# arangrhie/merfin

Measured on AMD Instinct MI355X. Metric: k-mers evaluated/sec (-hist, k=21), higher is better.
Workload: dtype u64 k-mers / u32 counts / f64 K*

## Files before the change

### merfin_amd/csrc/mfx_device.h

```cpp
#pragma once
#include "mfx_internal.h"
#include "mfx_kernels.h"

__device__ __forceinline__ uint64_t mfx_hash64(uint64_t x) {
  x ^= x >> 33; x *= 0xff51afd7ed558ccdULL;
  x ^= x >> 33; x *= 0xc4ceb9fe1a85ec53ULL;
  x ^= x >> 33;
  return x;
}

__device__ __forceinline__ uint32_t mfx_range32(uint64_t x, uint64_t n) {
  const uint32_t n32 = (uint32_t)n;
  const uint64_t t = (uint64_t)(uint32_t)(x >> 32) * n32 + (uint64_t)__umulhi((uint32_t)x, n32);
  return (uint32_t)(t >> 32);
}

__device__ __forceinline__ uint64_t mfx_field_mask(uint32_t nbits) { return nbits >= 64u ? ~0ull : (1ull << nbits) - 1ull; }
__device__ __forceinline__ uint64_t mfx_bits_at(const uint64_t *w, uint64_t bit, uint32_t nbits, uint64_t mask) {
  const uint64_t i = bit >> 6;
  const uint32_t sh = (uint32_t)bit & 63u;
  uint64_t x = w[i] >> sh;
  if (sh + nbits > 64u) x |= w[i + 1] << (64u - sh);
  return x & mask;
}
// ... 36 lines not shown

constexpr uint32_t MFX_TILE_BYTES  = MFX_TILE + 64;
constexpr uint32_t MFX_TILE_CHUNKS = MFX_TILE_BYTES / 16;
constexpr uint32_t MFX_TILE_WORDS  = MFX_TILE_BYTES / 32;

struct mfx_tile_lds {
  uint64_t codes[MFX_TILE_WORDS + 1];
  uint32_t valid[MFX_TILE_WORDS + 1];
};

__device__ __forceinline__ void mfx_pack16(uint4 v, uint32_t &codes, uint32_t &valid) {
  uint32_t w[4] = {v.x, v.y, v.z, v.w};
  codes = 0;
  valid = 0;
#pragma unroll
  for (int q = 0; q < 4; ++q) {
#pragma unroll
    for (int b = 0; b < 4; ++b) {
      uint32_t c = (w[q] >> (8 * b)) & 0xffu;
      uint32_t u = (c & 0xDFu) - 0x41u;
      uint32_t ok = (u < 32u) ? ((0x00080045u >> u) & 1u) : 0u;
      int i = q * 4 + b;
      codes |= ((c >> 1) & 3u) << (30 - 2 * i);
      valid |= ok << (15 - i);
    }
  }
}

__device__ __forceinline__ void mfx_tile_fill(mfx_tile_lds &L, const uint8_t *__restrict__ src) {
  uint32_t *c32 = reinterpret_cast<uint32_t *>(L.codes);
  uint16_t *v16 = reinterpret_cast<uint16_t *>(L.valid);
  for (uint32_t ch = threadIdx.x; ch < MFX_TILE_CHUNKS; ch += MFX_BLOCK) {
    uint4 v = *reinterpret_cast<const uint4 *>(src + 16ull * ch);
    uint32_t codes, valid;
    mfx_pack16(v, codes, valid);
    c32[ch ^ 1] = codes;
    v16[ch ^ 1] = (uint16_t)valid;
  }
}

__device__ __forceinline__ void mfx_tile_fill_packed(mfx_tile_lds &L, const uint64_t *__restrict__ codes, const uint32_t *__restrict__ valid) {
  for (uint32_t i = threadIdx.x; i < MFX_TILE_WORDS; i += MFX_BLOCK) {
    L.codes[i] = codes[i];
    L.valid[i] = valid[i];
  }
}

__device__ __forceinline__ uint64_t mfx_wave_sum(uint64_t v) {
#pragma unroll
  for (int o = 32; o > 0; o >>= 1) v += __shfl_down(v, o, 64);
  return v;
}

__device__ __forceinline__ void mfx_block_sum3(uint64_t &a, uint64_t &b, uint64_t &c, uint64_t (*scratch)[3]) {
  a = mfx_wave_sum(a); b = mfx_wave_sum(b); c = mfx_wave_sum(c);
  uint32_t wave = threadIdx.x >> 6, lane = threadIdx.x & 63;
  __syncthreads();
  if (lane == 0) { scratch[wave][0] = a; scratch[wave][1] = b; scratch[wave][2] = c; }
  __syncthreads();
  if (threadIdx.x == 0) {
    a = b = c = 0;
    for (uint32_t w = 0; w < MFX_BLOCK / 64; ++w) { a += scratch[w][0]; b += scratch[w][1]; c += scratch[w][2]; }
  }
}


#ifndef MFX_V_LDS_DIET
#define MFX_V_LDS_DIET 1
#endif
struct mfx_hist_lds {
  uint32_t hist[2 * MFX_NB_LDS];
  uint32_t rk[MFX_MAXP_LDS];
#if !MFX_V_LDS_DIET
  double   pr[MFX_MAXP_LDS];
#endif
  uint16_t bin[MFX_KLUT * MFX_KLUT];
#if !MFX_V_LDS_DIET
  double   term[MFX_KLUT * MFX_KLUT];
#endif
  uint32_t lut_ok;
  uint32_t wl_n;
  uint64_t next[2];
  uint64_t tot[2];
  uint64_t red[MFX_BLOCK / 64][3];
  double   dred[MFX_BLOCK];
};

__device__ __forceinline__ void mfx_hist_lds_init(mfx_hist_lds &H, const mfx_kstar_args &ka) {
  const uint32_t tid = threadIdx.x;
  for (uint32_t i = tid; i < 2 * MFX_NB_LDS; i += MFX_BLOCK) H.hist[i] = 0;
  if (tid == 0) H.lut_ok = 1u;
  __syncthreads();
  for (uint32_t v = tid; v < MFX_MAXP_LDS; v += MFX_BLOCK) {
    double rk, pr;
    mfx_getK_core(ka.peak, ka.n_prob, ka.probK, ka.probP, v, rk, pr);
    if (!(rk >= 0.0 && rk < 4294967296.0 && rk == (double)(uint32_t)rk)) H.lut_ok = 0u;
    H.rk[v] = (uint32_t)rk;
#if !MFX_V_LDS_DIET
    H.pr[v] = pr;
#endif
  }
  for (uint32_t i = tid; i < MFX_KLUT * MFX_KLUT; i += MFX_BLOCK) {
    uint32_t h = i / MFX_KLUT, l = i % MFX_KLUT;
    uint32_t b = (h >= 1 && l >= 1 && h >= l) ? mfx_bin_index((double)h, (double)l) : 0u;
    H.bin[i] = (uint16_t)b;
#if !MFX_V_LDS_DIET
    H.term[i] = (h >= 1 && l >= 1 && h > l) ? mfx_overcopy_term((double)l, (double)h, 1.0) : 0.0;
#endif
  }
  __syncthreads();
}

__device__ __forceinline__ void mfx_ovf_add(uint64_t *ovf, uint64_t key, uint64_t amount) {
  unsigned long long *cnt = reinterpret_cast<unsigned long long *>(ovf) + 2, *keys = cnt + MFX_OVF_SLOTS;
  uint64_t x = key * 0x9E3779B97F4A7C15ull;
  uint32_t h = (uint32_t)(x >> 40) & (MFX_OVF_SLOTS - 1u);
  for (uint32_t probe = 0; probe < MFX_OVF_PROBES; ++probe) {
    unsigned long long cur = __hip_atomic_load(&keys[h], __ATOMIC_RELAXED, __HIP_MEMORY_SCOPE_AGENT);
    if (cur == ~0ull) {
      cur = atomicCAS(&keys[h], ~0ull, (unsigned long long)key);
      if (cur == ~0ull) { atomicAdd(reinterpret_cast<unsigned long long *>(ovf), 1ull); cur = key; }
    }
    if (cur == key) { atomicAdd(&cnt[h], (unsigned long long)amount); return; }
    h = (h + 1u) & (MFX_OVF_SLOTS - 1u);
  }
  atomicAdd(reinterpret_cast<unsigned long long *>(ovf) + 1, (unsigned long long)amount);
}

__device__ __forceinline__ void mfx_ovf_record(const mfx_kstar_args &ka, bool under, uint32_t idx) {
  const uint64_t key = (under ? 0ull : (1ull << 63)) | idx;
  const uint32_t lane = threadIdx.x & 63u;
  uint64_t todo = __ballot(1);
  while (todo) {
    const int leader = __ffsll((unsigned long long)todo) - 1;
    const uint64_t lk = ((uint64_t)(uint32_t)__shfl((int)(key >> 32), leader, 64) << 32) | (uint32_t)__shfl((int)(uint32_t)key, leader, 64);
    const uint64_t same = __ballot(key == lk) & todo;
    if ((int)lane == leader) {
      const uint64_t n = (uint64_t)__popcll(same);
      mfx_ovf_add(ka.ovf, key, n);
      atomicAdd((unsigned long long *)&ka.counts[2ull * ka.nbins + 2], (unsigned long long)n);
    }
    todo &= ~same;
  }
}

template <class Counter>
__device__ __forceinline__ bool mfx_hist_eval(mfx_hist_lds &H, const mfx_kstar_args &ka, bool lut_ok, uint32_t readV,
                                              uint32_t asmV, Counter &n_over0, double &kover) {
  double readK, prob;
  uint32_t rki = 0xffffffffu;
  if (lut_ok && readV < MFX_MAXP_LDS) {
#if MFX_V_LDS_DIET
    rki = H.rk[readV]; prob = 1.0; readK = (double)rki;
#else
    rki = H.rk[readV]; prob = H.pr[readV]; readK = (double)rki;
#endif
  } else {
    mfx_getK_core(ka.peak, ka.n_prob, ka.probK, ka.probP, readV, readK, prob);
  }
  const double asmK = (double)asmV;
  if (readK == 0) return true;
  const bool under = asmK > readK;
  uint32_t idx;
  if (rki < MFX_KLUT && asmV < MFX_KLUT && asmV >= 1) {
    const uint32_t hi = under ? asmV : rki, lo = under ? rki : asmV;
    idx = H.bin[hi * MFX_KLUT + lo];
// ... 77 lines not shown
```

### merfin_amd/csrc/mfx_kernels.hip

```cpp
#include "mfx_internal.h"
#include "mfx_kernels.h"
#include "mfx_device.h"
#include "mfx_place.h"
#include "mfx_track.h"
#define MFX_REGIONS_DEVICE
#include "mfx_regions.h"
#include "mfx_spectrum.h"

#include <stdlib.h>
#include <algorithm>

__device__ __forceinline__ uint64_t mfx_revcomp(uint64_t fwd, int k) {
  uint64_t x = __brevll(fwd) >> (64 - 2 * k);
  x = ((x & 0x5555555555555555ULL) << 1) | ((x >> 1) & 0x5555555555555555ULL);
  uint64_t mask = (~0ULL) >> (64 - 2 * k);
  return (x ^ 0xAAAAAAAAAAAAAAAAULL) & mask;
}


constexpr uint32_t MFX_MZ_REGION = 4;
constexpr uint32_t MFX_MAX_LINES = 512;

struct mfx_probe {
  uint32_t lineA, lineB;
// ... 1555 lines not shown
      }
      if (have) x = make_uint2((r_rv < c.minV || r_rv > c.maxV) ? 0u : r_rv, r_av);
#pragma unroll
      for (int j = 0; j < B; ++j)
        if (sj == j) { rv[j] = x.x; av[j] = x.y; st[j] = 0xffu; }
    }
  }
  return defer;
}

template <class KmerAt, class Eval, class Push1>
__device__ __forceinline__ void mfx_lane_flush(const mfx_table_view &c, mfx_mailbox &M, uint32_t &nq, KmerAt kmer_at, Eval eval, Push1 push1, unsigned long long *dbg = nullptr) {
  const uint32_t tid = threadIdx.x, sub16 = (tid & 7u) << 4, lane = tid & 63u, wbase = tid & ~63u;
  const uint32_t n = nq;
  nq = 0u;
  if (n == 0u) return;
  mfx_wave_handoff();
  constexpr uint32_t STEPS = 4;
  auto tail_pass = [&](bool second) {
    for (uint32_t q0 = 0; q0 < n; q0 += 8u * STEPS) {
      uint4 sl[STEPS];
      uint32_t fl[STEPS];
      bool act[STEPS];
#pragma unroll
      for (uint32_t sp = 0; sp < STEPS; ++sp) {
        const uint32_t e = q0 + 8u * sp + (lane >> 3);
        sl[sp] = make_uint4(0u, 0u, 0u, 0u);
        act[sp] = false;
        fl[sp] = 0u;
        if (e < n) {
          const uint2 lw = *reinterpret_cast<const uint2 *>(reinterpret_cast<const uint32_t *>(&M.rec[wbase + e]) + 2);
          fl[sp] = lw.y;
          act[sp] = lw.x != MFX_REC_FOUND && (!second || (lw.y & 3u) == 2u);
          if (act[sp]) sl[sp] = *reinterpret_cast<const uint4 *>(reinterpret_cast<uint64_t>(c.slots) + ((uint64_t)lw.x << 7) + sub16);
        }
      }
      mfx_wave_handoff();
#pragma unroll
      for (uint32_t sp = 0; sp < STEPS; ++sp) {
        const uint32_t e = q0 + 8u * sp + (lane >> 3);
        if (act[sp]) {
          uint32_t *rec = reinterpret_cast<uint32_t *>(&M.rec[wbase + e]);
          const uint2 kk = *reinterpret_cast<const uint2 *>(rec);
          if (sl[sp].y == 0xffffffffu || sl[sp].w == 0xffffffffu) rec[3] = (fl[sp] & ~3u) | 1u;
          if (sl[sp].y == kk.y && ((sl[sp].x ^ kk.x) >> 22) == 0u) { rec[0] = sl[sp].x; rec[2] = MFX_REC_FOUND; }
          else if (sl[sp].w == kk.y && ((sl[sp].z ^ kk.x) >> 22) == 0u) { rec[0] = sl[sp].z; rec[2] = MFX_REC_FOUND; }
        }
      }
    }
    mfx_wave_handoff();
  };
  tail_pass(false);
  const bool mine = lane < n;
  uint4 r = make_uint4(0u, 0u, MFX_REC_FOUND, 0u);
  if (mine) r = M.rec[wbase + lane];
  const bool full = mine && r.z != MFX_REC_FOUND && (r.w & 3u) != 1u;
  if (__any(full)) {
    if (full) {
      uint32_t *rec = reinterpret_cast<uint32_t *>(&M.rec[wbase + lane]);
      mfx_probe pr;
      pr.lineA = pr.lineB = r.z;
      rec[2] = (uint32_t)mfx_probe_line(c, pr, 1u);
      rec[3] = (r.w & ~3u) | 2u;
      if (c.quot) rec[1] = r.y | (1u << (MFX_Q_DSHIFT + 22 - 32));
      if (dbg) atomicAdd(&dbg[1], 1ull);
    }
    mfx_wave_handoff();
    tail_pass(true);
    if (full) {
      const uint4 r2 = M.rec[wbase + lane];
      r.x = r2.x; r.w = r2.w;
      if (r2.z == MFX_REC_FOUND) r.z = MFX_REC_FOUND;
    }
  }
  bool have = r.z == MFX_REC_FOUND;
  uint32_t lo = r.x;
  uint64_t fk = (((uint64_t)r.y << 32) | r.x) >> 22;
  if (c.quot) fk &= (1ull << MFX_Q_DSHIFT) - 1ull;
  const bool scan = mine && !have && (r.w & 3u) == 2u;
  const bool satd = mine && have && (((lo >> 11) & MFX_CSAT) == MFX_CSAT || (lo & MFX_CSAT) == MFX_CSAT);
  bool listed = false;
  if (__any(scan || satd)) {
    if (dbg && (scan || satd)) atomicAdd(&dbg[scan ? 3 : 2], 1ull);
    listed = push1(scan || satd, (scan || satd) ? (c.quot ? kmer_at(r.w >> 4) : fk) : 0ull, scan ? r.z : lo, scan ? 1u : 2u) && (scan || satd);
  }
  if (mine && !listed) {
    bool beyond = false;
    if (scan) {
      if (dbg) atomicAdd(&dbg[5], 1ull);
      const uint2 fd = mfx_c_find_lean(c, fk, r.z, 2u, beyond);
      have = fd.x != 0u;
      lo = fd.y;
    }
    uint32_t r_rv = (lo >> 11) & MFX_CSAT, r_av = lo & MFX_CSAT;
    const bool sat = have && (r_rv == MFX_CSAT || r_av == MFX_CSAT);
    if (sat || beyond) {
      const uint2 sx = mfx_side_lookup_lean(c, c.quot ? kmer_at(r.w >> 4) : fk);
      if (beyond) { r_rv = sx.x; r_av = sx.y; have = true; }
      else { if (r_rv == MFX_CSAT) r_rv = sx.x; if (r_av == MFX_CSAT) r_av = sx.y; }
    }
    uint32_t o_rv = 0u, o_av = 0u;
    if (have) { o_rv = (r_rv < c.minV || r_rv > c.maxV) ? 0u : r_rv; o_av = r_av; }
    eval(o_rv, o_av);
  }
  mfx_wave_handoff();
}

template <int B>
struct mfx_key_from_array {
  const uint64_t (&key)[B];
  __device__ __forceinline__ uint64_t operator()(int sj) const {
    uint64_t k = 0;
#pragma unroll
    for (int j = 0; j < B; ++j) if (j == sj) k = key[j];
    return k;
  }
};

#ifndef MFX_V_LANEPROBE
#define MFX_V_LANEPROBE 1
#endif

template <int B>
__device__ __forceinline__ void mfx_compact_lookup(const mfx_table_view &t, mfx_mailbox &M, const uint64_t (&key)[B], const uint64_t (&krc)[B],
                                                   const bool (&ok)[B], uint32_t (&rv)[B], uint32_t (&av)[B]) {
#if MFX_V_LANEPROBE
  uint64_t fkey[B];
  uint32_t line[B], b0[B];
#pragma unroll
  for (int j = 0; j < B; ++j) {
    fkey[j] = key[j]; line[j] = 0u; b0[j] = 0u;
    if (ok[j]) { const mfx_probe pr = mfx_home(t, key[j]); fkey[j] = pr.fkey; line[j] = pr.lineA; b0[j] = pr.b0; }
  }
  (void)mfx_lane_lookup8<B>(t, M, fkey, ok, rv, av, line, b0, mfx_key_from_array<B>{key});
#else
  mfx_group_lookup8<B>(t, M, key, krc, ok, rv, av);
#endif
}
#define MFX_COMPACT_LOOKUP(t, MB, key, krc, ok, rv, av) mfx_compact_lookup<MFX_BATCH>(t, MB, key, krc, ok, rv, av)

__device__ __forceinline__ bool mfx_tile_kmer(const mfx_tile_lds &L, int k, uint32_t p, uint64_t &fwd) {
  uint32_t w = p >> 5, o = p & 31;
  uint64_t w0 = L.codes[w], w1 = L.codes[w + 1];
  uint32_t sh = 2 * o;
  uint64_t hi = (w0 << sh) | ((w1 >> 1) >> (63 - sh));
  fwd = hi >> (64 - 2 * k);
  uint64_t vv = (((uint64_t)L.valid[w] << 32) | L.valid[w + 1]) << o;
  return (vv >> (64 - k)) == ((~0ULL) >> (64 - k));
}

#ifndef MFX_V_MIN2LEVEL
#define MFX_V_MIN2LEVEL 1
#endif
typedef unsigned short mfx_us2 __attribute__((ext_vector_type(2)));
__device__ __forceinline__ uint32_t mfx_pk_min_u16(uint32_t a, uint32_t b) {
  return __builtin_bit_cast(uint32_t, __builtin_elementwise_min(__builtin_bit_cast(mfx_us2, a), __builtin_bit_cast(mfx_us2, b)));
}
__device__ __forceinline__ uint32_t mfx_mod_pack(uint32_t order, uint32_t q) { return ((order << 7) | q) | (((order << 7) | (127u - q)) << 16); }

template <int B>
__device__ __forceinline__ void mfx_wave_mod_halo(const mfx_table_view &c, const mfx_tile_lds &L, uint32_t p0, uint32_t (&halo)[2]) {
  const int t = c.mz_t;
  const uint32_t H = (uint32_t)(c.k - t), per = 64u / H;
  const uint32_t lane = threadIdx.x & 63u;
  const uint32_t jj = lane / H, ii = lane - H * jj;
#pragma unroll
  for (uint32_t ps = 0; ps < 2u; ++ps) {
    halo[ps] = 0xffffffffu;
    const uint32_t el = ps * per + jj;
    if (ps * per < (uint32_t)B && jj < per && el < (uint32_t)B) {
      const uint32_t q = p0 - lane + el * MFX_BLOCK + 64u + ii, wd = q >> 5, o = q & 31u, sh = 2u * o;
      const uint64_t w0 = L.codes[wd], w1 = L.codes[wd + 1];
      const uint32_t a = (uint32_t)(((w0 << sh) | ((w1 >> 1) >> (63u - sh))) >> (64 - 2 * t));
      const uint32_t b = (uint32_t)mfx_revcomp((uint64_t)a, t);
      halo[ps] = mfx_mod_pack(mfx_tmer_order(a < b ? a : b), 64u + ii);
    }
  }
}

__device__ __forceinline__ uint32_t mfx_wave_mod_line(const mfx_table_view &c, uint32_t *mw, const uint32_t (&halo)[2], int j, uint64_t f, uint64_t r,
                                                      uint32_t &b0, uint64_t &fkey) {
  const int k = c.k, t = c.mz_t, w = c.mz_w, m = k - w + 1, npos = k - t + 1;
  const uint32_t lane = threadIdx.x & 63u, tmask = (1u << (2 * t)) - 1u;
  const uint32_t H = (uint32_t)(k - t), per = 64u / H;
  const uint64_t mmask = (~0ULL) >> (64 - 2 * m);
  const uint32_t a = (uint32_t)(f >> (2 * (k - t))) & tmask, b = (uint32_t)r & tmask;
  const uint32_t hsrc = (uint32_t)j < per ? halo[0] : halo[1];
  const uint32_t hv = (uint32_t)__shfl((int)hsrc, (int)(H * ((uint32_t)j < per ? (uint32_t)j : (uint32_t)j - per) + lane), 64);
  mfx_wave_handoff();
  mw[lane] = mfx_mod_pack(mfx_tmer_order(a < b ? a : b), lane);
  if (lane <= H) mw[64u + lane] = lane < H ? hv : 0xffffffffu;
  mfx_wave_handoff();
  uint32_t v = 0xffffffffu;
#if MFX_V_MIN2LEVEL
  {
    const int g1 = npos >= 26 ? 6 : npos >= 10 ? 4 : npos >= 5 ? 3 : 2, g2 = (npos + g1 - 1) / g1;
    uint32_t a0 = 0xffffffffu, a1 = 0xffffffffu;
#pragma unroll
    for (int i = 0; i < 6; ++i)
      if (i < g1) { a0 = mfx_pk_min_u16(a0, mw[lane + (uint32_t)i]); a1 = mfx_pk_min_u16(a1, mw[(lane <= (uint32_t)(npos - g1) ? 64u + lane : lane) + (uint32_t)i]); }
    mfx_wave_handoff();
    mw[lane] = a0;
    if (lane <= (uint32_t)(npos - g1)) mw[64u + lane] = a1;
    mfx_wave_handoff();
#pragma unroll
    for (int j = 0; j < 7; ++j)
      if (j < g2) v = mfx_pk_min_u16(v, mw[lane + (uint32_t)(j * g1 < npos - g1 ? j * g1 : npos - g1)]);
  }
#else
#pragma unroll
  for (int i = 0; i < 28; ++i)
    if (i < npos) v = mfx_pk_min_u16(v, mw[lane + (uint32_t)i]);
#endif
  const bool fwd = f <= r;
  const uint32_t q = fwd ? (v & 127u) : 127u - ((v >> 16) & 127u);
  const uint32_t xf = q - lane, jf = xf % (uint32_t)w;
  const uint64_t ma = (f >> (2 * ((uint32_t)w - 1u - jf))) & mmask, mb = (r >> (2 * jf)) & mmask;
  const uint32_t xc = fwd ? xf : (uint32_t)(k - t) - xf;
  uint32_t line;
  fkey = fwd ? f : r;
  if (c.quot) {
    const uint32_t jc = fwd ? jf : 3u - jf;
    const uint64_t ac = fwd ? ma : mb, bc = fwd ? mb : ma;
    const uint32_t e = (uint32_t)(((fkey >> (2 * (m + 3 - (int)jc))) << (2 * (3 - (int)jc))) | (fkey & ((1ull << (2 * (3 - (int)jc))) - 1ull)));
    mfx_q_place(c, ac < bc ? ac : bc, bc < ac ? 1u : 0u, jc, e, xc, line, b0, fkey);
  } else {
    const bool lt = ma < mb, keep = lt || (fwd && ma == mb);
    mfx_mod_place(lt ? ma : mb, keep ? jf : (uint32_t)w - 1u - jf, c.nlines, line, b0, xc);
  }
  return line;
}


#ifndef MFX_V_BATCH
#define MFX_V_BATCH 4
#endif
constexpr int MFX_BATCH = MFX_V_BATCH;

#ifndef MFX_V_MINBLOCKS
#define MFX_V_MINBLOCKS 4
#endif
#ifndef MFX_V_MINBLOCKS_K21
#define MFX_V_MINBLOCKS_K21 7
#endif
#ifndef MFX_V_BATCH_K21
#define MFX_V_BATCH_K21 2
#endif
#ifndef MFX_V_MINBLOCKS_K31
#define MFX_V_MINBLOCKS_K31 6
#endif
#ifndef MFX_V_BATCH_K31
#define MFX_V_BATCH_K31 2
#endif
#ifndef MFX_V_MINBLOCKS_GEN
#define MFX_V_MINBLOCKS_GEN 4
#endif
#ifndef MFX_V_BATCH_GEN
#define MFX_V_BATCH_GEN 4
#endif
#ifndef MFX_V_DEFER_K21
#define MFX_V_DEFER_K21 0
#endif
#ifndef MFX_V_DEFER_K31
#define MFX_V_DEFER_K31 1
#endif
#ifndef MFX_V_KFXLDS_K21
#define MFX_V_KFXLDS_K21 1
#endif
constexpr uint32_t MFX_KFX_BASE = 32u;
#ifndef MFX_V_BUCKET2_K21
#define MFX_V_BUCKET2_K21 0
#endif
#ifndef MFX_V_BUCKET2_K31
#define MFX_V_BUCKET2_K31 1
#endif
template <bool CANON, bool COMPACT, int KF> struct mfx_hist_tune { static constexpr int blocks = MFX_V_MINBLOCKS, batch = MFX_V_BATCH, defer = 0, kfxlds = 0, bucket2 = 0; };
template <> struct mfx_hist_tune<true, true, 21> { static constexpr int blocks = MFX_V_MINBLOCKS_K21, batch = MFX_V_BATCH_K21, defer = MFX_V_DEFER_K21, kfxlds = MFX_V_KFXLDS_K21, bucket2 = MFX_V_BUCKET2_K21; };
#ifndef MFX_V_KFXLDS_K31
#define MFX_V_KFXLDS_K31 0
#endif
template <> struct mfx_hist_tune<true, true, 31> { static constexpr int blocks = MFX_V_MINBLOCKS_K31, batch = MFX_V_BATCH_K31, defer = MFX_V_DEFER_K31, kfxlds = MFX_V_KFXLDS_K31, bucket2 = MFX_V_BUCKET2_K31; };
template <> struct mfx_hist_tune<true, true, 0> { static constexpr int blocks = MFX_V_MINBLOCKS_GEN, batch = MFX_V_BATCH_GEN, defer = 0, kfxlds = 0, bucket2 = 0; };
template <bool CANON, bool COMPACT, int KF, int WF, int TF, bool DBG = false>
__global__ __launch_bounds__(MFX_BLOCK, (mfx_hist_tune<CANON, COMPACT, KF>::blocks)) void mfx_hist_kernel(mfx_hist_args a) {
  constexpr int BT = mfx_hist_tune<CANON, COMPACT, KF>::batch;
  __shared__ mfx_tile_lds L;
  __shared__ mfx_mailbox MB;
  __shared__ mfx_hist_lds H;

  const uint32_t tid = threadIdx.x;
  if (KF) { a.t.k = KF; a.t.mz_w = WF; a.t.mz_t = TF; a.t.quot = KF > MFX_MAX_K_DIRECT ? 1 : 0; }
  const int k = KF ? KF : a.t.k;
  const mfx_kstar_args &ka = a.ks;
  mfx_hist_lds_init(H, ka);
  const bool lut_ok = H.lut_ok != 0u;

  uint32_t n_valid = 0, n_missing = 0, n_over0 = 0;
  if (tid == 0) { H.tot[0] = H.tot[1] = 0; H.wl_n = 0u; }
  uint64_t *c_glob = ka.counts + 2ull * ka.nbins;
  uint64_t *c_kasm = c_glob + 3, *c_kmis = c_kasm + ka.ncontigs;

  const uint32_t none = 0xffffffffu;
  uint32_t c = none;
  uint64_t li = blockIdx.x;
  for (uint32_t it = 0; li < a.n_logical; ++it) {
    if (tid == 0)
      H.next[it & 1] = (uint64_t)gridDim.x + atomicAdd((unsigned long long *)a.tile_ctr, 1ull);
    const uint64_t tile = a.part_n == 1 ? a.tile_begin + li
                                         : ((((li >> a.part_shift) * a.part_n + a.part_rank) << a.part_shift) | (li & ((1ull << a.part_shift) - 1ull)));
    const uint32_t cn = a.tile_contig[tile];
    if (cn != c) {
      if (c != none) {
        uint64_t x = n_valid, y = n_missing, z = 0;
        mfx_block_sum3(x, y, z, H.red);
        if (tid == 0 && (x | y)) {
          atomicAdd((unsigned long long *)&c_kasm[c], x);
          atomicAdd((unsigned long long *)&c_kmis[c], y);
          H.tot[0] += x;
          H.tot[1] += y;
        }
        n_valid = n_missing = 0;
      }
      c = cn;
    }
    const uint64_t pos0 = (tile - a.tile_start[c]) * MFX_TILE;
    const uint64_t clen = a.contig_len[c];
    const uint32_t n = (clen - pos0 < MFX_TILE) ? (uint32_t)(clen - pos0) : MFX_TILE;
    const uint8_t *src = a.bases + a.contig_off[c] + pos0;

    if (a.codes) {
      const uint64_t w0 = (a.contig_off[c] + pos0) >> 5;
      mfx_tile_fill_packed(L, a.codes + w0, a.valid + w0);
    } else {
      mfx_tile_fill(L, src);
    }
    __syncthreads();

    uint64_t kfx = 0;
    constexpr bool kfx_lds = mfx_hist_tune<CANON, COMPACT, KF>::kfxlds != 0 && COMPACT && CANON && KF != 0 && TF != 0;
    constexpr uint32_t mb_cap = kfx_lds ? MFX_KFX_BASE : 64u;
    static_assert(!(mfx_hist_tune<CANON, COMPACT, KF>::kfxlds != 0 && mfx_hist_tune<CANON, COMPACT, KF>::defer != 0),
                  "kfxlds packs 16 terms and a count of at most 16 into one LDS word per lane: the deferred probe lets a lane evaluate more than its own 16 k-mers of a tile");
    static_assert(MFX_TILE / MFX_BLOCK <= 16, "the packed koverCpy word (56-bit sum, 8-bit count) holds 16 evaluations per lane and tile");
    unsigned long long *const kfxw = reinterpret_cast<unsigned long long *>(&MB.rec[(tid & ~63u) + MFX_KFX_BASE]) + (tid & 63u);
    if (kfx_lds) *kfxw = 0ull;
    struct lds_bump { unsigned long long *w; __device__ __forceinline__ void operator++(int) { (void)__hip_atomic_fetch_add(reinterpret_cast<uint32_t *>(w) + 1, 1u << 24, __ATOMIC_RELAXED, __HIP_MEMORY_SCOPE_WORKGROUP); } };
    struct lds_sum { unsigned long long *w; __device__ __forceinline__ void operator+=(uint64_t v) { (void)__hip_atomic_fetch_add(w, (unsigned long long)v, __ATOMIC_RELAXED, __HIP_MEMORY_SCOPE_WORKGROUP); } };
    auto eval1 = [&](uint32_t rvv, uint32_t avv) {
      if (kfx_lds) {
        lds_bump bump{kfxw};
        lds_sum sum{kfxw};
        if (mfx_hist_eval_fx(H, ka, lut_ok, rvv, avv, bump, sum)) n_missing++;
      } else if (mfx_hist_eval_fx(H, ka, lut_ok, rvv, avv, n_over0, kfx)) n_missing++;
    };
    const bool wave_lines = COMPACT && CANON && (KF ? TF != 0 : a.t.mz_t != 0);
    const bool defer_tail = MFX_V_DEFER != 0 && mfx_hist_tune<CANON, COMPACT, KF>::defer != 0 && COMPACT && CANON && KF != 0 && TF != 0 && (KF & 1) != 0;
    const bool quotf = KF ? KF > MFX_MAX_K_DIRECT : a.t.quot != 0;
    constexpr bool bucket2 = MFX_V_BUCKET2 != 0 && mfx_hist_tune<CANON, COMPACT, KF>::bucket2 != 0;
    auto push_wave = [&](bool want, uint64_t kmer, uint32_t aux, uint32_t mode, bool dbl) -> bool {
      if (!a.wl) return false;
      const uint64_t m = __ballot(want);
      if (!m) return false;
      const uint32_t ln = tid & 63u, leader = (uint32_t)__ffsll((unsigned long long)m) - 1u;
      uint32_t base = 0;
      if (ln == leader) base = atomicAdd(&H.wl_n, (uint32_t)__popcll(m));
      base = (uint32_t)__shfl((int)base, (int)leader, 64);
      const uint32_t at = base + (uint32_t)__popcll(m & ((1ULL << ln) - 1ULL));
      const bool fits = want && at < a.wl_segcap;
      if (fits) reinterpret_cast<uint4 *>(a.wl + MFX_WL_HEADER)[(uint64_t)blockIdx.x * a.wl_segcap + at] =
                  make_uint4((uint32_t)kmer, (uint32_t)(kmer >> 32), aux, ((uint32_t)li * (MFX_BLOCK / 64) + (tid >> 6)) | (dbl ? 0x80000000u : 0u) | (mode << 29));
      return fits;
    };
    uint32_t nq = 0;
    uint32_t *const mwave = reinterpret_cast<uint32_t *>(H.dred) + (tid >> 6) * 128u;
    for (uint32_t b = 0;; b += BT) {
      const bool last = b >= MFX_TILE / MFX_BLOCK || b * MFX_BLOCK >= n;
      nq = (uint32_t)__builtin_amdgcn_readfirstlane((int)nq);
      if (defer_tail && (last || nq >= (MFX_DEFER_FLUSH < mb_cap ? MFX_DEFER_FLUSH : mb_cap / 2u))) {
        auto kmer_at = [&](uint32_t p) -> uint64_t {
          uint64_t f;
          (void)mfx_tile_kmer(L, k, p, f);
          const uint64_t r = mfx_revcomp(f, k);
          return f < r ? f : r;
        };
        mfx_lane_flush(a.t, MB, nq, kmer_at, eval1, [&](bool want, uint64_t km, uint32_t aux, uint32_t mode) { return push_wave(want, km, aux, mode, false); }, DBG ? reinterpret_cast<unsigned long long *>(a.dbg) : nullptr);
      }
      if (last) break;
      uint32_t rv[BT], av[BT];
      bool     ok[BT];
      uint32_t parked = 0u;
      const bool even_k = KF ? (KF & 1) == 0 : (k & 1) == 0;
      if (wave_lines) {
        uint64_t fkey[BT];
        uint32_t line[BT], b0[BT];
        uint32_t halo[2], pal = 0u;
        mfx_wave_mod_halo<BT>(a.t, L, b * MFX_BLOCK + tid, halo);
#pragma unroll
        for (int j = 0; j < BT; ++j) {
          const uint32_t p = (b + j) * MFX_BLOCK + tid;
          uint64_t f;
          ok[j] = mfx_tile_kmer(L, k, p, f) && (p < n);
          const uint64_t r = mfx_revcomp(f, k);
          line[j] = mfx_wave_mod_line(a.t, mwave, halo, j, f, r, b0[j], fkey[j]);
          if (!ok[j]) { line[j] = 0u; b0[j] = 0u; }
          if (even_k && f == r) pal |= 1u << j;
        }
        const bool quot = quotf;
        auto keyof = [&](int sj) -> uint64_t {
          uint64_t kk = 0;
          if (!quot) {
#pragma unroll
            for (int j = 0; j < BT; ++j) if (j == sj) kk = fkey[j];
          } else {
            uint64_t f;
            (void)mfx_tile_kmer(L, k, (b + (uint32_t)sj) * MFX_BLOCK + tid, f);
            const uint64_t r = mfx_revcomp(f, k);
            kk = f < r ? f : r;
          }
          return kk;
        };
        if (defer_tail) {
          uint32_t posn[BT];
#pragma unroll
          for (int j = 0; j < BT; ++j) posn[j] = (b + (uint32_t)j) * MFX_BLOCK + tid;
          auto pj = [&](int jj, bool want, uint64_t km, uint32_t aux, uint32_t mode) { (void)jj; return push_wave(want, km, aux, mode, false); };
          parked = mfx_lane_probe_defer<BT, decltype(keyof), mfx_push_fn<decltype(pj)>, mb_cap, bucket2>(
                       a.t, MB, nq, fkey, ok, rv, av, line, b0, posn, keyof, DBG ? reinterpret_cast<unsigned long long *>(a.dbg) : nullptr, mfx_push_fn<decltype(pj)>{pj});
        } else {
          auto pj = [&](int jj, bool want, uint64_t km, uint32_t aux, uint32_t mode) { return push_wave(want, km, aux, mode, ((pal >> jj) & 1u) != 0u); };
          parked = mfx_lane_lookup8<BT, decltype(keyof), mfx_push_fn<decltype(pj)>, mb_cap, bucket2>(
                       a.t, MB, fkey, ok, rv, av, line, b0, keyof, DBG ? reinterpret_cast<unsigned long long *>(a.dbg) : nullptr, mfx_push_fn<decltype(pj)>{pj});
        }
        if (even_k) {
#pragma unroll
          for (int j = 0; j < BT; ++j) if ((pal >> j) & 1u) { rv[j] += rv[j]; av[j] += av[j]; }
        }
      } else {
        uint64_t key[BT], key2[BT];
#pragma unroll
        for (int j = 0; j < BT; ++j) {
          const uint32_t p = (b + j) * MFX_BLOCK + tid;
          uint64_t f;
          ok[j] = mfx_tile_kmer(L, k, p, f) && (p < n);
          const uint64_t r = mfx_revcomp(f, k);
          if (CANON) {
            key[j] = f < r ? f : r; key2[j] = f < r ? r : f;
          } else {
            key[j] = f; key2[j] = r;
          }
        }
        if (COMPACT) mfx_compact_lookup<BT>(a.t, MB, key, key2, ok, rv, av);
        else mfx_group_lookup<BT>(a.t, MB, key, key2, ok, rv, av);
        if (!CANON) {
          uint32_t rv2[BT], av2[BT];
          if (COMPACT) mfx_compact_lookup<BT>(a.t, MB, key2, key, ok, rv2, av2);
          else mfx_group_lookup<BT>(a.t, MB, key2, key, ok, rv2, av2);
#pragma unroll
          for (int j = 0; j < BT; ++j) { rv[j] += rv2[j]; av[j] += av2[j]; }
        } else if (even_k) {
#pragma unroll
          for (int j = 0; j < BT; ++j) if (key[j] == key2[j]) { rv[j] += rv[j]; av[j] += av[j]; }
        }
      }
#pragma unroll
      for (int j = 0; j < BT; ++j) {
        if (!ok[j]) continue;
        n_valid++;
        if (!((parked >> j) & 1u)) eval1(rv[j], av[j]);
      }
    }
    if (kfx_lds) { mfx_wave_handoff(); const unsigned long long w = *kfxw; kfx = w & ((1ull << 56) - 1ull); n_over0 += (uint32_t)(w >> 56); }
#pragma unroll
    for (int off = 32; off > 0; off >>= 1) kfx += __shfl_down(kfx, off, 64);
    if ((tid & 63u) == 0) reinterpret_cast<uint64_t *>(a.tile_partials)[li * (MFX_BLOCK / 64) + (tid >> 6)] = kfx;

    __syncthreads();
    const uint64_t nx = H.next[it & 1];
    li = ((uint64_t)__builtin_amdgcn_readfirstlane((uint32_t)(nx >> 32)) << 32) |
         (uint64_t)__builtin_amdgcn_readfirstlane((uint32_t)nx);
  }
  {
    uint64_t x = n_valid, y = n_missing, z = n_over0;
    mfx_block_sum3(x, y, z, H.red);
    if (tid == 0 && a.wl) a.wl[2 + blockIdx.x] = H.wl_n < a.wl_segcap ? H.wl_n : a.wl_segcap;
    if (tid == 0) {
      if (c != none && (x | y)) {
        atomicAdd((unsigned long long *)&c_kasm[c], x);
        atomicAdd((unsigned long long *)&c_kmis[c], y);
      }
      if (H.tot[0] + x) atomicAdd((unsigned long long *)&c_glob[0], H.tot[0] + x);
      if (H.tot[1] + y) atomicAdd((unsigned long long *)&c_glob[1], H.tot[1] + y);
      if (z) atomicAdd((unsigned long long *)&ka.counts[ka.nbins], z);
    }
  }
  mfx_hist_lds_flush_bins(H, ka);
}

constexpr uint32_t MFX_REST_SPLIT = 4;
__global__ __launch_bounds__(MFX_BLOCK) void mfx_hist_rest_kernel(mfx_hist_args a) {
  __shared__ mfx_hist_lds H;
  const uint32_t tid = threadIdx.x;
  const mfx_kstar_args &ka = a.ks;
  uint64_t *c_glob = ka.counts + 2ull * ka.nbins, *c_kmis = c_glob + 3 + ka.ncontigs;
  uint64_t *kfx_words = reinterpret_cast<uint64_t *>(a.tile_partials);
  uint32_t n_missing = 0, n_over0 = 0;
  bool ready = false, lut_ok = false;
  for (uint32_t sb = blockIdx.x; sb < a.wl_segs * MFX_REST_SPLIT; sb += gridDim.x) {
    const uint32_t seg = sb / MFX_REST_SPLIT, part = sb % MFX_REST_SPLIT;
    const uint32_t n = (uint32_t)__hip_atomic_load(reinterpret_cast<unsigned long long *>(&a.wl[2 + seg]), __ATOMIC_RELAXED, __HIP_MEMORY_SCOPE_AGENT);
    if (n <= part * MFX_BLOCK) continue;
    if (!ready) { mfx_hist_lds_init(H, ka); lut_ok = H.lut_ok != 0u; ready = true; }
    const uint4 *ent = reinterpret_cast<const uint4 *>(a.wl + MFX_WL_HEADER) + (uint64_t)seg * a.wl_segcap;
    for (uint32_t i0 = part * MFX_BLOCK; i0 < n; i0 += MFX_REST_SPLIT * MFX_BLOCK) {
      const uint32_t i = i0 + tid;
      const bool live = i < n;
      uint4 e = make_uint4(0u, 0u, 0u, 0u);
      if (live) e = ent[i];
      bool missing = false;
      if (live) {
        const uint64_t km = ((uint64_t)e.y << 32) | e.x;
        uint2 x = make_uint2(0u, 0u);
        const uint32_t mode = (e.w >> 29) & 3u;
        if (mode == 2u) x = mfx_c_fields(a.t, km, e.z);
        else if (!a.t.quot) {
          mfx_probe pr;
          pr.lineA = e.z; pr.lineB = a.t.mz_w > 0 ? mfx_range32(mfx_hash64(km), a.t.nlines) : e.z; pr.b0 = 0u; pr.fkey = km;
          unsigned long long word = 0;
          bool beyond;
          if (mfx_c_find(a.t, pr, mode == 1u ? 2u : 0u, word, beyond)) x = mfx_c_fields(a.t, km, (uint32_t)word);
        } else x = mfx_c_lookup(a.t, km);
        if (e.w >> 31) { x.x += x.x; x.y += x.y; }
        uint64_t kfx = 0;
        missing = mfx_hist_eval_fx(H, ka, lut_ok, x.x, x.y, n_over0, kfx);
        if (kfx) atomicAdd(reinterpret_cast<unsigned long long *>(&kfx_words[e.w & 0x1fffffffu]), (unsigned long long)kfx);
      }
      uint32_t ctg = 0u;
      if (missing) {
        const uint64_t li = (e.w & 0x1fffffffu) / (MFX_BLOCK / 64);
        const uint64_t tile = a.part_n == 1 ? a.tile_begin + li
                                             : ((((li >> a.part_shift) * a.part_n + a.part_rank) << a.part_shift) | (li & ((1ull << a.part_shift) - 1ull)));
        ctg = a.tile_contig[tile];
      }
      uint64_t todo = __ballot(missing);
      while (todo) {
        const int leader = __ffsll((unsigned long long)todo) - 1;
        const uint32_t lc = (uint32_t)__shfl((int)ctg, leader, 64);
        const uint64_t same = __ballot(missing && ctg == lc) & todo;
        if ((int)(tid & 63u) == leader) atomicAdd(reinterpret_cast<unsigned long long *>(&c_kmis[lc]), (unsigned long long)__popcll(same));
        todo &= ~same;
      }
      if (missing) n_missing++;
    }
  }
  if (!ready) return;
  {
    uint64_t x = 0, y = n_missing, z = n_over0;
    mfx_block_sum3(x, y, z, H.red);
    if (tid == 0) {
      if (y) atomicAdd(reinterpret_cast<unsigned long long *>(&c_glob[1]), (unsigned long long)y);
// ... 1514 lines not shown
```

Before: 154.4 billion.

## Assign contiguous k-mer runs per wave and accumulate K* terms in shared LDS slots

Changes the k-mer-to-thread mapping so each wave processes contiguous 64-position runs (wave-major cells) instead of a block-strided layout, and passes the position/slot through flush, push and eval paths. K* term sums are accumulated with LDS atomics into per-slot words rather than per-lane registers followed by a wave shuffle reduction, and per-tile partials are written from those slots after the barrier. Also replaces __shfl with a direct ds_bpermute for the halo exchange. The aim is better locality of the tile codes and minimizer halos and removal of the per-tile reduction, at the cost of contended LDS atomics on a few shared words.

```diff
diff --git a/merfin_amd/csrc/mfx_device.h b/merfin_amd/csrc/mfx_device.h
--- a/merfin_amd/csrc/mfx_device.h
+++ b/merfin_amd/csrc/mfx_device.h
@@ -142,6 +142,7 @@
   uint32_t wl_n;
   uint64_t next[2];
   uint64_t tot[2];
+  unsigned long long kfx_slot[MFX_BLOCK / 64];
   uint64_t red[MFX_BLOCK / 64][3];
   double   dred[MFX_BLOCK];
 };
diff --git a/merfin_amd/csrc/mfx_kernels.hip b/merfin_amd/csrc/mfx_kernels.hip
--- a/merfin_amd/csrc/mfx_kernels.hip
+++ b/merfin_amd/csrc/mfx_kernels.hip
@@ -1661,7 +1661,7 @@
   bool listed = false;
   if (__any(scan || satd)) {
     if (dbg && (scan || satd)) atomicAdd(&dbg[scan ? 3 : 2], 1ull);
-    listed = push1(scan || satd, (scan || satd) ? (c.quot ? kmer_at(r.w >> 4) : fk) : 0ull, scan ? r.z : lo, scan ? 1u : 2u) && (scan || satd);
+    listed = push1(scan || satd, (scan || satd) ? (c.quot ? kmer_at(r.w >> 4) : fk) : 0ull, scan ? r.z : lo, scan ? 1u : 2u, r.w >> 4) && (scan || satd);
   }
   if (mine && !listed) {
     bool beyond = false;
@@ -1680,7 +1680,7 @@
     }
     uint32_t o_rv = 0u, o_av = 0u;
     if (have) { o_rv = (r_rv < c.minV || r_rv > c.maxV) ? 0u : r_rv; o_av = r_av; }
-    eval(o_rv, o_av);
+    eval(o_rv, o_av, r.w >> 4);
   }
   mfx_wave_handoff();
 }
@@ -1738,7 +1738,7 @@
 __device__ __forceinline__ uint32_t mfx_mod_pack(uint32_t order, uint32_t q) { return ((order << 7) | q) | (((order << 7) | (127u - q)) << 16); }
 
 template <int B>
-__device__ __forceinline__ void mfx_wave_mod_halo(const mfx_table_view &c, const mfx_tile_lds &L, uint32_t p0, uint32_t (&halo)[2]) {
+__device__ __forceinline__ void mfx_wave_mod_halo(const mfx_table_view &c, const mfx_tile_lds &L, uint32_t p0, uint32_t stride, uint32_t (&halo)[2]) {
   const int t = c.mz_t;
   const uint32_t H = (uint32_t)(c.k - t), per = 64u / H;
   const uint32_t lane = threadIdx.x & 63u;
@@ -1748,7 +1748,7 @@
     halo[ps] = 0xffffffffu;
     const uint32_t el = ps * per + jj;
     if (ps * per < (uint32_t)B && jj < per && el < (uint32_t)B) {
-      const uint32_t q = p0 - lane + el * MFX_BLOCK + 64u + ii, wd = q >> 5, o = q & 31u, sh = 2u * o;
+      const uint32_t q = p0 - lane + el * stride + 64u + ii, wd = q >> 5, o = q & 31u, sh = 2u * o;
       const uint64_t w0 = L.codes[wd], w1 = L.codes[wd + 1];
       const uint32_t a = (uint32_t)(((w0 << sh) | ((w1 >> 1) >> (63u - sh))) >> (64 - 2 * t));
       const uint32_t b = (uint32_t)mfx_revcomp((uint64_t)a, t);
@@ -1765,7 +1765,7 @@
   const uint64_t mmask = (~0ULL) >> (64 - 2 * m);
   const uint32_t a = (uint32_t)(f >> (2 * (k - t))) & tmask, b = (uint32_t)r & tmask;
   const uint32_t hsrc = (uint32_t)j < per ? halo[0] : halo[1];
-  const uint32_t hv = (uint32_t)__shfl((int)hsrc, (int)(H * ((uint32_t)j < per ? (uint32_t)j : (uint32_t)j - per) + lane), 64);
+  const uint32_t hv = (uint32_t)__builtin_amdgcn_ds_bpermute((int)((H * ((uint32_t)j < per ? (uint32_t)j : (uint32_t)j - per) + lane) << 2), (int)hsrc);
   mfx_wave_handoff();
   mw[lane] = mfx_mod_pack(mfx_tmer_order(a < b ? a : b), lane);
   if (lane <= H) mw[64u + lane] = lane < H ? hv : 0xffffffffu;
@@ -1860,6 +1860,12 @@
 #endif
 template <> struct mfx_hist_tune<true, true, 31> { static constexpr int blocks = MFX_V_MINBLOCKS_K31, batch = MFX_V_BATCH_K31, defer = MFX_V_DEFER_K31, kfxlds = MFX_V_KFXLDS_K31, bucket2 = MFX_V_BUCKET2_K31; };
 template <> struct mfx_hist_tune<true, true, 0> { static constexpr int blocks = MFX_V_MINBLOCKS_GEN, batch = MFX_V_BATCH_GEN, defer = 0, kfxlds = 0, bucket2 = 0; };
+template <int BT>
+__device__ __forceinline__ uint32_t mfx_hist_cell(uint32_t wv, uint32_t j) { return wv * (uint32_t)BT + j; }
+template <int BT>
+__device__ __forceinline__ uint32_t mfx_hist_pos(uint32_t b, uint32_t wv, uint32_t tid, uint32_t j) { return b * MFX_BLOCK + (mfx_hist_cell<BT>(wv, j) << 6) + (tid & 63u); }
+template <int BT>
+__device__ __forceinline__ uint32_t mfx_hist_slot(uint32_t wv, uint32_t j) { return mfx_hist_cell<BT>(wv, j) & (MFX_BLOCK / 64 - 1u); }
 template <bool CANON, bool COMPACT, int KF, int WF, int TF, bool DBG = false>
 __global__ __launch_bounds__(MFX_BLOCK, (mfx_hist_tune<CANON, COMPACT, KF>::blocks)) void mfx_hist_kernel(mfx_hist_args a) {
   constexpr int BT = mfx_hist_tune<CANON, COMPACT, KF>::batch;
@@ -1868,6 +1874,7 @@
   __shared__ mfx_hist_lds H;
 
   const uint32_t tid = threadIdx.x;
+  const uint32_t wv = (uint32_t)__builtin_amdgcn_readfirstlane((int)(tid >> 6));
   if (KF) { a.t.k = KF; a.t.mz_w = WF; a.t.mz_t = TF; a.t.quot = KF > MFX_MAX_K_DIRECT ? 1 : 0; }
   const int k = KF ? KF : a.t.k;
   const mfx_kstar_args &ka = a.ks;
@@ -1876,6 +1883,7 @@
 
   uint32_t n_valid = 0, n_missing = 0, n_over0 = 0;
   if (tid == 0) { H.tot[0] = H.tot[1] = 0; H.wl_n = 0u; }
+  if (tid < MFX_BLOCK / 64) H.kfx_slot[tid] = 0ull;
   uint64_t *c_glob = ka.counts + 2ull * ka.nbins;
   uint64_t *c_kasm = c_glob + 3, *c_kmis = c_kasm + ka.ncontigs;
 
@@ -1915,28 +1923,28 @@
     }
     __syncthreads();
 
-    uint64_t kfx = 0;
     constexpr bool kfx_lds = mfx_hist_tune<CANON, COMPACT, KF>::kfxlds != 0 && COMPACT && CANON && KF != 0 && TF != 0;
     constexpr uint32_t mb_cap = kfx_lds ? MFX_KFX_BASE : 64u;
     static_assert(!(mfx_hist_tune<CANON, COMPACT, KF>::kfxlds != 0 && mfx_hist_tune<CANON, COMPACT, KF>::defer != 0),
-                  "kfxlds packs 16 terms and a count of at most 16 into one LDS word per lane: the deferred probe lets a lane evaluate more than its own 16 k-mers of a tile");
-    static_assert(MFX_TILE / MFX_BLOCK <= 16, "the packed koverCpy word (56-bit sum, 8-bit count) holds 16 evaluations per lane and tile");
+                  "kfxlds keeps a count of at most 16 in 8 bits of one LDS word per lane: the deferred probe lets a lane evaluate more than its own 16 k-mers of a tile");
+    static_assert(MFX_TILE / MFX_BLOCK <= 16, "the lane's word (an 8-bit count of the dominant bin) holds 16 evaluations per lane and tile");
+    static_assert(MFX_TILE / (MFX_BLOCK / 64) <= 1024, "a slot's word holds the terms (at most 2^52 units each) of 1024 positions of a tile");
     unsigned long long *const kfxw = reinterpret_cast<unsigned long long *>(&MB.rec[(tid & ~63u) + MFX_KFX_BASE]) + (tid & 63u);
     if (kfx_lds) *kfxw = 0ull;
     struct lds_bump { unsigned long long *w; __device__ __forceinline__ void operator++(int) { (void)__hip_atomic_fetch_add(reinterpret_cast<uint32_t *>(w) + 1, 1u << 24, __ATOMIC_RELAXED, __HIP_MEMORY_SCOPE_WORKGROUP); } };
     struct lds_sum { unsigned long long *w; __device__ __forceinline__ void operator+=(uint64_t v) { (void)__hip_atomic_fetch_add(w, (unsigned long long)v, __ATOMIC_RELAXED, __HIP_MEMORY_SCOPE_WORKGROUP); } };
-    auto eval1 = [&](uint32_t rvv, uint32_t avv) {
+    auto eval1 = [&](uint32_t rvv, uint32_t avv, uint32_t slot) {
+      lds_sum sum{&H.kfx_slot[slot]};
       if (kfx_lds) {
         lds_bump bump{kfxw};
-        lds_sum sum{kfxw};
         if (mfx_hist_eval_fx(H, ka, lut_ok, rvv, avv, bump, sum)) n_missing++;
-      } else if (mfx_hist_eval_fx(H, ka, lut_ok, rvv, avv, n_over0, kfx)) n_missing++;
+      } else if (mfx_hist_eval_fx(H, ka, lut_ok, rvv, avv, n_over0, sum)) n_missing++;
     };
     const bool wave_lines = COMPACT && CANON && (KF ? TF != 0 : a.t.mz_t != 0);
     const bool defer_tail = MFX_V_DEFER != 0 && mfx_hist_tune<CANON, COMPACT, KF>::defer != 0 && COMPACT && CANON && KF != 0 && TF != 0 && (KF & 1) != 0;
     const bool quotf = KF ? KF > MFX_MAX_K_DIRECT : a.t.quot != 0;
     constexpr bool bucket2 = MFX_V_BUCKET2 != 0 && mfx_hist_tune<CANON, COMPACT, KF>::bucket2 != 0;
-    auto push_wave = [&](bool want, uint64_t kmer, uint32_t aux, uint32_t mode, bool dbl) -> bool {
+    auto push_wave = [&](bool want, uint64_t kmer, uint32_t aux, uint32_t mode, bool dbl, uint32_t slot) -> bool {
       if (!a.wl) return false;
       const uint64_t m = __ballot(want);
       if (!m) return false;
@@ -1947,7 +1955,7 @@
       const uint32_t at = base + (uint32_t)__popcll(m & ((1ULL << ln) - 1ULL));
       const bool fits = want && at < a.wl_segcap;
       if (fits) reinterpret_cast<uint4 *>(a.wl + MFX_WL_HEADER)[(uint64_t)blockIdx.x * a.wl_segcap + at] =
-                  make_uint4((uint32_t)kmer, (uint32_t)(kmer >> 32), aux, ((uint32_t)li * (MFX_BLOCK / 64) + (tid >> 6)) | (dbl ? 0x80000000u : 0u) | (mode << 29));
+                  make_uint4((uint32_t)kmer, (uint32_t)(kmer >> 32), aux, ((uint32_t)li * (MFX_BLOCK / 64) + slot) | (dbl ? 0x80000000u : 0u) | (mode << 29));
       return fits;
     };
     uint32_t nq = 0;
@@ -1962,7 +1970,8 @@
           const uint64_t r = mfx_revcomp(f, k);
           return f < r ? f : r;
         };
-        mfx_lane_flush(a.t, MB, nq, kmer_at, eval1, [&](bool want, uint64_t km, uint32_t aux, uint32_t mode) { return push_wave(want, km, aux, mode, false); }, DBG ? reinterpret_cast<unsigned long long *>(a.dbg) : nullptr);
+        auto eval_at = [&](uint32_t rvv, uint32_t avv, uint32_t p) { eval1(rvv, avv, (p >> 6) & (MFX_BLOCK / 64 - 1u)); };
+        mfx_lane_flush(a.t, MB, nq, kmer_at, eval_at, [&](bool want, uint64_t km, uint32_t aux, uint32_t mode, uint32_t p) { return push_wave(want, km, aux, mode, false, (p >> 6) & (MFX_BLOCK / 64 - 1u)); }, DBG ? reinterpret_cast<unsigned long long *>(a.dbg) : nullptr);
       }
       if (last) break;
       uint32_t rv[BT], av[BT];
@@ -1973,10 +1982,10 @@
         uint64_t fkey[BT];
         uint32_t line[BT], b0[BT];
         uint32_t halo[2], pal = 0u;
-        mfx_wave_mod_halo<BT>(a.t, L, b * MFX_BLOCK + tid, halo);
+        mfx_wave_mod_halo<BT>(a.t, L, mfx_hist_pos<BT>(b, wv, tid, 0u), 64u, halo);
 #pragma unroll
         for (int j = 0; j < BT; ++j) {
-          const uint32_t p = (b + j) * MFX_BLOCK + tid;
+          const uint32_t p = mfx_hist_pos<BT>(b, wv, tid, (uint32_t)j);
           uint64_t f;
           ok[j] = mfx_tile_kmer(L, k, p, f) && (p < n);
           const uint64_t r = mfx_revcomp(f, k);
@@ -1992,7 +2001,7 @@
             for (int j = 0; j < BT; ++j) if (j == sj) kk = fkey[j];
           } else {
             uint64_t f;
-            (void)mfx_tile_kmer(L, k, (b + (uint32_t)sj) * MFX_BLOCK + tid, f);
+            (void)mfx_tile_kmer(L, k, mfx_hist_pos<BT>(b, wv, tid, (uint32_t)sj), f);
             const uint64_t r = mfx_revcomp(f, k);
             kk = f < r ? f : r;
           }
@@ -2001,12 +2010,12 @@
         if (defer_tail) {
           uint32_t posn[BT];
 #pragma unroll
-          for (int j = 0; j < BT; ++j) posn[j] = (b + (uint32_t)j) * MFX_BLOCK + tid;
-          auto pj = [&](int jj, bool want, uint64_t km, uint32_t aux, uint32_t mode) { (void)jj; return push_wave(want, km, aux, mode, false); };
+          for (int j = 0; j < BT; ++j) posn[j] = mfx_hist_pos<BT>(b, wv, tid, (uint32_t)j);
+          auto pj = [&](int jj, bool want, uint64_t km, uint32_t aux, uint32_t mode) { return push_wave(want, km, aux, mode, false, mfx_hist_slot<BT>(wv, (uint32_t)jj)); };
           parked = mfx_lane_probe_defer<BT, decltype(keyof), mfx_push_fn<decltype(pj)>, mb_cap, bucket2>(
                        a.t, MB, nq, fkey, ok, rv, av, line, b0, posn, keyof, DBG ? reinterpret_cast<unsigned long long *>(a.dbg) : nullptr, mfx_push_fn<decltype(pj)>{pj});
         } else {
-          auto pj = [&](int jj, bool want, uint64_t km, uint32_t aux, uint32_t mode) { return push_wave(want, km, aux, mode, ((pal >> jj) & 1u) != 0u); };
+          auto pj = [&](int jj, bool want, uint64_t km, uint32_t aux, uint32_t mode) { return push_wave(want, km, aux, mode, ((pal >> jj) & 1u) != 0u, mfx_hist_slot<BT>(wv, (uint32_t)jj)); };
           parked = mfx_lane_lookup8<BT, decltype(keyof), mfx_push_fn<decltype(pj)>, mb_cap, bucket2>(
                        a.t, MB, fkey, ok, rv, av, line, b0, keyof, DBG ? reinterpret_cast<unsigned long long *>(a.dbg) : nullptr, mfx_push_fn<decltype(pj)>{pj});
         }
@@ -2018,7 +2027,7 @@
         uint64_t key[BT], key2[BT];
 #pragma unroll
         for (int j = 0; j < BT; ++j) {
-          const uint32_t p = (b + j) * MFX_BLOCK + tid;
+          const uint32_t p = mfx_hist_pos<BT>(b, wv, tid, (uint32_t)j);
           uint64_t f;
           ok[j] = mfx_tile_kmer(L, k, p, f) && (p < n);
           const uint64_t r = mfx_revcomp(f, k);
@@ -2045,15 +2054,16 @@
       for (int j = 0; j < BT; ++j) {
         if (!ok[j]) continue;
         n_valid++;
-        if (!((parked >> j) & 1u)) eval1(rv[j], av[j]);
-      }
-    }
-    if (kfx_lds) { mfx_wave_handoff(); const unsigned long long w = *kfxw; kfx = w & ((1ull << 56) - 1ull); n_over0 += (uint32_t)(w >> 56); }
-#pragma unroll
-    for (int off = 32; off > 0; off >>= 1) kfx += __shfl_down(kfx, off, 64);
-    if ((tid & 63u) == 0) reinterpret_cast<uint64_t *>(a.tile_partials)[li * (MFX_BLOCK / 64) + (tid >> 6)] = kfx;
+        if (!((parked >> j) & 1u)) eval1(rv[j], av[j], mfx_hist_slot<BT>(wv, (uint32_t)j));
+      }
+    }
+    if (kfx_lds) { mfx_wave_handoff(); n_over0 += (uint32_t)(*kfxw >> 56); }
 
     __syncthreads();
+    if (tid < MFX_BLOCK / 64) {
+      reinterpret_cast<uint64_t *>(a.tile_partials)[li * (MFX_BLOCK / 64) + tid] = H.kfx_slot[tid];
+      H.kfx_slot[tid] = 0ull;
+    }
     const uint64_t nx = H.next[it & 1];
     li = ((uint64_t)__builtin_amdgcn_readfirstlane((uint32_t)(nx >> 32)) << 32) |
          (uint64_t)__builtin_amdgcn_readfirstlane((uint32_t)nx);
```

Result: faster. 156.7 billion (median of 6 runs) (+1.5%).
